# adaliaramon/LambdaGap

Hardware: AMD Instinct MI355X
Metric: boosting iters/sec + AUC, synthetic Higgs-shape 10M×28, 255 bins, 63 leaves (higher is better)
Workload: dtype fp32; 1 GPU; model=gbdt binary, 63 leaves, 255 bins, lr 0.1, global_batch=10000000, seq_len=28, parallelism=dp1, device=AMD GPU (gfx950:sramecc+:xnack-) [frontier engine]

## Files before the change

### src/device/device_learner.hip

```cpp
#include <hip/hip_runtime.h>

#include <algorithm>
#include <chrono>
#include <cmath>
#include <cstdio>
#include <cstdlib>
#include <cstring>
#include <fstream>
#include <map>
#include <memory>
#include <string>
#include <vector>

#include "device/grad_kernels.h"
#include "device/hip_common.h"
#include "device/leaf_kernels.h"
#include "device/metric_eval.h"
#include "device/linear_kernels.h"
#include "device/runtime_internal.h"
#include "device/frontier.h"
#include "device/policy_scan.h"
#include "device/traverse_kernels.h"
#include "device/sample_kernels.h"
#include "device/engine_plan.h"
#include "device/seq_kernels.h"
#include "device/split_scan.h"
#include "device/tree_kernels.h"
#include "learner/forced_splits.h"
#include "learner/linear_solve.h"
#include "learner/parallel_tree_learner.h"
#include "learner/serial_tree_learner.h"
#include "lgap/common.h"
#include "lgap/device_api.h"
#include "lgap/network.h"
#include "lgap/objective.h"
#include "lgap/rank_math.h"
#include "lgap/metric.h"
#include "lgap/split_math.h"

namespace lgap {
namespace device {
namespace {

const char* KernelOverride(const char* key) {
  static const char* const kKeys[] = {"fhist_threads", "hist_lds_kb", "quant_lds32", "part_iters",
                                      "hist_il",       "nibble",      "quant_hist",  "scan_global",
                                      "scan_wave",     "oob_rows",    "select_merge", "part_grid"};
  constexpr int kNumKeys = static_cast<int>(sizeof(kKeys) / sizeof(kKeys[0]));
  thread_local std::string vals[kNumKeys];
  const char* e = std::getenv("LGAP_KERNEL");
  if (e == nullptr) return nullptr;
  const std::string s(e);
  const char* found = nullptr;
  for (size_t p = 0; p < s.size();) {
    size_t q = s.find(',', p);
    if (q == std::string::npos) q = s.size();
    const std::string item = s.substr(p, q - p);
    p = q + 1;
    if (item.empty()) continue;
    const size_t eq = item.find('=');
    const std::string k = item.substr(0, eq);
    int idx = -1;
    for (int i = 0; i < kNumKeys; ++i) idx = k == kKeys[i] ? i : idx;
    if (idx < 0) Log::Fatal("LGAP_KERNEL: unknown key '%s'", k.c_str());
    if (k == key) {
      vals[idx] = eq == std::string::npos ? "1" : item.substr(eq + 1);
      found = vals[idx].c_str();
    }
  }
  return found;
}


using namespace seq;

class DeviceTreeLearner : public TreeLearner {
 public:
  DeviceTreeLearner(const Config* config, const std::string& learner_type, bool routed = false)
      : config_(config), learner_type_(learner_type), routed_(routed) {}

  ~DeviceTreeLearner() override {
    if (fres_host_) (void)hipHostFree(fres_host_);
    if (graph_exec_) (void)hipGraphExecDestroy(graph_exec_);
    for (auto& kv : fgraphs_) (void)hipGraphExecDestroy(kv.second);
    if (fcont_) (void)hipGraphExecDestroy(fcont_);
    if (!fx_peers_.empty()) XgmiClose(fx_local_, &fx_peers_);
    if (fx_local_) (void)hipFree(fx_local_);
    for (auto& ev : pipe_ev_) {
      if (ev) (void)hipEventDestroy(ev);
    }
    if (comm_stream_) (void)hipStreamDestroy(comm_stream_);
    if (stream_) (void)hipStreamDestroy(stream_);
  }

  void Init(const Dataset* train, bool is_constant_hessian) override {
    is_const_hess_ = is_constant_hessian;
    data_ = train;
    N_ = train->num_data();
    F_ = train->num_features();
    G_ = train->num_groups();
    TB_ = train->num_total_bin();
    width_ = train->bin_width();
    stride_dw_ = train->row_stride() / 4;
    tstride_dw_ = stride_dw_;
    if (learner_type_ != "serial" && !CommActive() && !HostStagedDP() && Network::num_machines() > 1) {
      Log::Fatal("Parallel HIP training needs an RCCL communicator (LGBM_DeviceCommInit)");
    }
    plan_in_ = PlanInputs();
    Replan();
    device_id_ = CommExists() ? CommDevice() : std::max(0, config_->gpu_device_id);
    HIP_CHECK(hipSetDevice(device_id_));
    hipDeviceProp_t prop;
    HIP_CHECK(hipGetDeviceProperties(&prop, device_id_));
    device_name_ = std::string(prop.name[0] ? prop.name : "AMD GPU") + " (" + prop.gcnArchName + ")";
    num_cu_ = prop.multiProcessorCount;
    if (!stream_) HIP_CHECK(hipStreamCreateWithFlags(&stream_, hipStreamNonBlocking));

    use_dp_ = config_->gpu_use_dp;
    UploadData();
    linear_ = config_->linear_tree;
    if (linear_) {
      if (!train->has_raw() && F_ > 0) {
        Log::Fatal("linear_tree requires the Dataset to keep raw feature values (construct it with linear_tree=true)");
      }
      const auto& raw = train->raw_values();
      lin_has_nan_ = false;
      for (float v : raw) {
        if (std::isnan(v)) {
          lin_has_nan_ = true;
          break;
// ... 1357 lines not shown
    a.L = L_;
    a.C = fC_;
    a.kmax = fkmax_;
    a.gstart = gstart_.get();
    a.feat = feat_.get();
    a.tiles = tiles_.get();
    a.num_tiles = num_tiles_;
    a.used_bytree = used_bytree_.get();
    a.tp = tparams_.get();
    a.st = fst_;
    a.nodes = fnodes_;
    a.exps = fexps_;
    a.exp_bits = fbits_;
    a.lsum = flsum_;
    a.lout = flout_;
    a.bounds = fbounds_;
    a.key = fkey_;
    a.best = fbest_;
    a.spl = fspl_;
    a.ic = use_ic_ ? fic_ : nullptr;
    a.ic_feat = use_ic_ ? fic_feat_.get() : nullptr;
    a.ic_words = ic_words_;
    a.nstate = fnst_;
    a.leaf_cid = flcid_;
    a.rec = rec_.get();
    a.range_out = range_.get();
    a.slots = fslots_.get();
    a.acc = reinterpret_cast<unsigned long long*>(facc_.get());
    a.hslab = fhslab_.get();
    a.hslab_stride = fhslab_stride_;
    a.hmeta = fhmeta_.get();
    a.red_grid = (num_tiles_ > 1 ? 4 : 2) * num_cu_;
    a.ghmax = ghmax_.get();
    a.sum_mult = plan_.distributed && !ffeature_ ? std::max(1, P_) : 1;
    {
      const char* e = std::getenv("LGAP_FIXED_SUMBOUND");
      a.sum_bound = e == nullptr || std::atoi(e) != 0;
    }
    a.forced = fnum_forced_ > 0 ? fforced_.get() : nullptr;
    a.num_forced = fnum_forced_;
    a.fbest = ffbest_;
    a.fkey = ffkey_;
    a.ckey = fckey_;
    a.cinfo = fcinfo_;
    a.tile_pub = ftile_pub_.get();
    a.bar = bar_.get();
    a.hist_min_rows = HistMinRows();
    a.hist_grid = FrontierHistBlocks();
    a.hist_threads = fhist_threads_;
    if (nib_) {
      a.rowbins = rowbins4_.get();
      a.stride_dw = stride4_dw_;
      a.tiles = ntile_.get();
      a.hist_nib = 1;
    }
    a.part_tile = fpart_tile_;
    a.max_depth = config_->max_depth;
    a.use_monotone = config_->monotone_constraints.empty() ? 0 : 1;
    a.mono_inter = fcbnd_ != nullptr ? 1 : 0;
    a.cbnd = fcbnd_;
    const char* sm = KernelOverride("select_merge");
    a.salive = sm != nullptr && sm[0] == '0' ? nullptr : fsal_;
    a.monotone_penalty = config_->monotone_penalty;
    a.cegb_split = CegbPenalty::Enabled(config_) ? config_->cegb_tradeoff * config_->cegb_penalty_split : 0.0;
    a.max_bin = max_bin_;
    a.cat_p2 = cat_p2_;
    a.use_dp = use_dp_ ? 1 : 0;
    a.ghq = ghq_.get();
    a.qmax = qmax_.get();
    a.quant = QuantHist() && ghq_.size() >= static_cast<size_t>(K_) * N_ ? 1 : 0;
    a.qbins = std::max(2, config_->num_grad_quant_bins);
    a.qconst = is_const_hess_ ? 1 : 0;
    {
      const double rows = static_cast<double>(N_);
      const double gl = a.qbins / 2, hl = a.qconst ? 1 : a.qbins;
      a.qpack = rows * gl < 2147483647.0 && rows * hl < 4294967295.0 ? 1 : 0;
      const int sub = static_cast<int>(std::min(32767.0 / gl, 65535.0 / hl));
      const char* e = KernelOverride("quant_lds32");
      const bool want = e != nullptr ? e[0] != '0' : num_tiles_ == 1;
      a.qsub = a.quant && !use_dp_ && sub >= 2048 && want ? sub : 0;
    }
    a.hist_il = !use_dp_ && a.qsub == 0 ? HistInterleave() : 0;
    {
      const bool fits = kFScanWaves * FrontierScanWaveBytes(max_bin_, cat_p2_) <= 150 * 1024;
      const char* sw = KernelOverride("scan_wave");
      a.scan_wave = fits && !has_cat_ && !a.mono_inter && (F_ >= 64 || (sw != nullptr && sw[0] == '1')) ? 1 : 0;
      a.scan_grid = 512;
    }
    a.e_lo = 0;
    a.e_hi = kFrontierKmax;
    if (plan_.raw_cands && fnuep_.size() > 0) {
      a.cegb_raw = 1;
      a.cegb_tradeoff = config_->cegb_tradeoff;
      a.nkey = fnkey_.get();
      a.ninfo = fninfo_.get();
      a.nuep = fnuep_.get();
      if (plan_.cegb_coupled) {
        a.cegb_coupled = cegb_coupled_.get();
        a.cegb_used = cegb_used_.get();
        a.cegb_epoch = cegb_epoch_.get();
      }
      if (plan_.cegb_lazy) {
        a.cegb_lazy = cegb_lazy_.get();
        a.lazy_bits = lazy_bits_.get();
        a.lazy_words = lazy_words_;
        a.lazy_acc = lazy_acc_.get();
        a.nlazy = fnlazy_.get();
        a.npath = fnpath_.get();
      }
    }
    a.spec_cap = fspec_cap_;
    a.policy = fpolicy_;
    a.stamps = fstamps_.size() ? fstamps_.get() : nullptr;
    a.distributed = plan_.distributed ? 1 : 0;
    a.kcap = fcaps_on_ ? fkcap_.get() : nullptr;
    a.kused = plan_.distributed ? fkused_.get() : nullptr;
    if (plan_.distributed) {
      const double gl = a.qbins / 2, hl = a.qconst ? 1 : a.qbins;
      a.qpack = fglobal_rows_ * gl < 2147483647.0 && fglobal_rows_ * hl < 4294967295.0 ? 1 : 0;
    }
    a.sp = MakeArgs().sp;
    a.bynode = use_bynode_ ? bynode_.get() : nullptr;
    a.byn_draw = frontier_ && plan_.bynode_on_device ? bynode_.get() : nullptr;
    a.byn_mode = fbyn_mode_.size() ? fbyn_mode_.get() : nullptr;
    a.byn_cnt = fbyn_cnt_;
    a.byn_reset = fbyn_reset_;
    a.xrng = config_->extra_trees ? rng_.get() : nullptr;
    if (ffeature_ || fowner_) {
      a.fowned = ffowned_.get();
      a.fpb = ffpb_.get();
      a.vote_P = P_;
      a.vote_rank = rank_;
      a.fown_list = fown_list_.get();
      a.fown_n = fown_n_;
    }
    a.xkb = fkmax_;
    if (fowner_) {
      a.own = 1;
      a.own_P = P_;
      a.own_rank = rank_;
      a.own_w = bbin_;
      a.own_b0 = fown_b0_.get();
      a.acc_recv = facc_recv_.get();
    }
    if (FrontierXg()) {
      a.xg = 1;
      a.xsession = 1;
      a.xc = fxconf_.get();
      if (fowner_ || ffeature_) a.fpb = reinterpret_cast<FPairBest*>(fx_local_ + fxo_fpb_);
      if (fowner_) a.acc_recv = reinterpret_cast<unsigned long long*>(fx_local_ + fxo_recv_);
    }
    if (fvoting_) {
      a.voting = 1;
      a.vote_k = topk_;
      a.vote_P = P_;
      a.vote_rank = rank_;
      a.sp_local = fsp_local_.get();
      a.lsum_loc = flsum_loc_.get();
      a.ltot = fltot_.get();
      a.vrec = fvrec_.get();
      a.velect = fvelect_.get();
      a.vrows = reinterpret_cast<unsigned long long*>(fvrows_.get());
      if (FrontierXg()) {
        a.vrec = reinterpret_cast<VoteRec*>(fx_local_ + fxo_vrec_);
        a.vrows = reinterpret_cast<unsigned long long*>(fx_local_ + fxo_vrows_);
      }
// ... 597 lines not shown
    for (int f = 0; f < F_; ++f) put(out + 8 * static_cast<size_t>(f), dev[f]);
    std::vector<float2> ghd(N_);
    HIP_CHECK(hipMemcpy(ghd.data(), gh_.get(), sizeof(float2) * N_, hipMemcpyDeviceToHost));
    std::vector<double> hg(N_), hh(N_);
    for (int i = 0; i < N_; ++i) {
      hg[i] = ghd[i].x;
      hh[i] = ghd[i].y;
    }
    double sg = 0.0, sh = 0.0;
    for (int i = 0; i < N_; ++i) {
      sg += hg[i];
      sh += hh[i];
    }
    const SplitParams sp = fa.sp;
    SplitParams p0 = sp;
    p0.path_smooth = 0.0;
    const double po = LeafOutputRaw(root_sum.x, root_sum.y, p0, N_, 0.0);
    for (int f = 0; f < F_; ++f) {
      const FeatureInfo& fi = data_->feature(f);
      std::vector<double> full(2 * static_cast<size_t>(fi.num_bin), 0.0);
      for (int i = 0; i < N_; ++i) {
        const uint32_t b = data_->FeatureBin(i, f);
        full[2 * b] += hg[i];
        full[2 * b + 1] += hh[i];
      }
      FeatureScanMeta m;
      m.num_bin = fi.num_bin;
      m.default_bin = fi.default_bin;
      m.missing_type = static_cast<int8_t>(fi.missing);
      m.bin_type = static_cast<int8_t>(fi.bin_type);
      m.monotone = fi.monotone;
      m.penalty = fi.penalty;
      SplitInfo r;
      r.Reset();
      bool ok;
      if (fi.bin_type == BinType::Numerical) {
        ok = FindBestNumerical(full.data(), m, sp, sg, sh, N_, po, LeafBounds(), &r);
      } else {
        std::vector<int> order(fi.num_bin);
        ok = FindBestCategorical(full.data(), m, sp, sg, sh, N_, po, LeafBounds(), order.data(), &r);
      }
      r.feature = ok ? f : -1;
      if (!ok) r.gain = kMinScore;
      put(ref + 8 * static_cast<size_t>(f), r);
    }
  }

  void TestFrontierHist(const float* g, const float* h, const int* rows, const int* offsets, int k, double* out,
                        uint16_t* levels) {
    if (!frontier_) Log::Fatal("TestFrontierHist: the frontier engine is not enabled for this configuration");
    if (k < 1 || k > fkmax_) Log::Fatal("TestFrontierHist: %d subsets (1..%d)", k, fkmax_);
    const int total = offsets[k];
    if (idx_[3].size() < static_cast<size_t>(total)) idx_[3].Resize(total);
    K_ = 1;
    DeviceSetGradients(g, h, 1);
    TreeParams* tp = pin_tp_.Get(1);
    std::memset(tp, 0, sizeof(TreeParams));
    tp->root_buf = -1;
    tp->root_count = tp->root_gcount = N_;
    tp->spec_alpha = 1.f;
    HIP_CHECK(hipMemcpyAsync(tparams_.get(), tp, sizeof(TreeParams), hipMemcpyHostToDevice, stream_));
    float bnd[4] = {0.f, 0.f, 0.f, 0.f};
    double sg = 0.0, sh = 0.0;
    for (int i = 0; i < N_; ++i) {
      bnd[0] = std::max(bnd[0], std::fabs(g[i]));
      bnd[1] = std::max(bnd[1], std::fabs(h[i]));
      sg += std::fabs(static_cast<double>(g[i]));
      sh += std::fabs(static_cast<double>(h[i]));
    }
    bnd[2] = std::nextafter(static_cast<float>(sg * (1.0 + 0x1p-20)), INFINITY);
    bnd[3] = std::nextafter(static_cast<float>(sh * (1.0 + 0x1p-20)), INFINITY);
    unsigned* hm = pin_max_.Get(4);
    std::memcpy(hm, bnd, 16);
    HIP_CHECK(hipMemcpyAsync(ghmax_.get(), hm, 16, hipMemcpyHostToDevice, stream_));
    if (config_->use_quantized_grad) QuantizeGradients(0);
    idx_[3].Upload(rows, total, stream_);
    FState st;
    std::memset(&st, 0, sizeof(st));
    st.round = 1;
    st.k = k;
    st.kx = k;
    st.num_leaves = 1;
    std::vector<FExp> ex(k);
    for (int e = 0; e < k; ++e) {
      std::memset(&ex[e], 0, sizeof(FExp));
      ex[e].h_buf = 3;
      ex[e].h_start = offsets[e];
      ex[e].h_count = offsets[e + 1] - offsets[e];
      ex[e].forced = -1;
    }
    HIP_CHECK(hipMemcpyAsync(fst_, &st, sizeof(FState), hipMemcpyHostToDevice, stream_));
    HIP_CHECK(hipMemcpyAsync(fexps_, ex.data(), sizeof(FExp) * k, hipMemcpyHostToDevice, stream_));
    facc_.Zero(stream_);
    FArgs fa = MakeFArgs();
    LaunchFrontierHist(fa, FrontierHistLds(), stream_);
    const int pw = fa.quant && fa.qpack ? 1 : 2;
    std::vector<unsigned long long> acc(static_cast<size_t>(k) * pw * TB_);
    HIP_CHECK(hipMemcpyAsync(acc.data(), facc_.get(), acc.size() * 8, hipMemcpyDeviceToHost, stream_));
    if (fa.quant && levels != nullptr) HIP_CHECK(hipMemcpyAsync(levels, ghq_.get(), sizeof(uint16_t) * N_, hipMemcpyDeviceToHost, stream_));
    HIP_CHECK(hipStreamSynchronize(stream_));
    facc_.Zero(stream_);
    HIP_CHECK(hipStreamSynchronize(stream_));
    constexpr double k62 = 4611686018427387904.0;
    const float sb2 = fa.sum_bound ? bnd[2] : INFINITY, sb3 = fa.sum_bound ? bnd[3] : INFINITY;
    const double ig = fa.quant ? 1.0 : std::ldexp(1.0, -FixedPointExp(k62, N_, bnd[0], sb2));
    const double ih = fa.quant ? 1.0 : std::ldexp(1.0, -FixedPointExp(k62, N_, bnd[1], sb3));
    for (int e = 0; e < k; ++e) {
      for (int b = 0; b < TB_; ++b) {
        const size_t o = (static_cast<size_t>(e) * TB_ + b) * pw;
        long long qg, qh;
        if (pw == 1) {
          const unsigned long long hs = acc[o] & 0xFFFFFFFFull;
          qg = static_cast<long long>(acc[o] - hs) >> 32;
          qh = static_cast<long long>(hs);
        } else {
          qg = static_cast<long long>(acc[o]);
          qh = static_cast<long long>(acc[o + 1]);
        }
        out[(static_cast<size_t>(e) * TB_ + b) * 2] = static_cast<double>(qg) * ig;
        out[(static_cast<size_t>(e) * TB_ + b) * 2 + 1] = static_cast<double>(qh) * ih;
      }
    }
  }

  bool TestQuantize(const float* g, const float* h, int num_class, int rounds, float* out_gh, uint16_t* out_levels,
                    uint32_t* out_qmax, float* out_true) {
    if (!config_->use_quantized_grad) Log::Fatal("TestQuantize: use_quantized_grad is not set");
    if (num_class < 1 || rounds < 1) Log::Fatal("TestQuantize: %d classes, %d rounds", num_class, rounds);
    K_ = num_class;
    const size_t n = static_cast<size_t>(N_);
    for (int r = 0; r < rounds; ++r) {
      DeviceSetGradients(g, h, num_class);
      for (int c = 0; c < num_class; ++c) {
        QuantizeGradients(c);
        const size_t o = (static_cast<size_t>(r) * num_class + c) * n;
        HIP_CHECK(hipMemcpyAsync(out_gh + 2 * o, gh_.get() + static_cast<size_t>(c) * n, sizeof(float2) * n,
                                 hipMemcpyDeviceToHost, stream_));
        if (QuantHist()) {
          HIP_CHECK(hipMemcpyAsync(out_levels + o, ghq_.get() + static_cast<size_t>(c) * n, sizeof(uint16_t) * n,
                                   hipMemcpyDeviceToHost, stream_));
        }
        HIP_CHECK(hipMemcpyAsync(out_qmax + 2 * (static_cast<size_t>(r) * num_class + c), qmax_.get(), 8,
                                 hipMemcpyDeviceToHost, stream_));
        if (config_->quant_train_renew_leaf) {
          HIP_CHECK(hipMemcpyAsync(out_true + 2 * o, gh_true_.get(), sizeof(float2) * n, hipMemcpyDeviceToHost, stream_));
        }
        HIP_CHECK(hipStreamSynchronize(stream_));
      }
    }
    return QuantHist();
  }

  void TestFrontierPartition(const int* rows, const int* offsets, int k, const int* feats, const int* thr,
                             const int* dleft, const uint32_t* catbits, int* out_rows, int* out_left, int* exp_rows,
                             int* exp_left) {
    if (!frontier_) Log::Fatal("TestFrontierPartition: the frontier engine is not enabled for this configuration");
    if (k < 1 || k > fkmax_ || 3 * k > fC_) Log::Fatal("TestFrontierPartition: %d parents (1..%d)", k, fkmax_);
    const int total = offsets[k];
    if (total > N_) Log::Fatal("TestFrontierPartition: %d rows over the subsets (at most %d)", total, N_);
    FState st;
    HIP_CHECK(hipMemcpyAsync(&st, fst_, sizeof(FState), hipMemcpyDeviceToHost, stream_));
    HIP_CHECK(hipStreamSynchronize(stream_));
    idx_[0].Upload(rows, total, stream_);
    std::vector<FExp> ex(k);
    std::vector<uint32_t> bits(static_cast<size_t>(fkmax_) * kMaxCatWords, 0u);
    int tiles = 0;
    for (int e = 0; e < k; ++e) {
      const int f = feats[e];
      if (f < 0 || f >= F_) Log::Fatal("TestFrontierPartition: feature %d", f);
      const FeatureInfo& fi = data_->feature(f);
      FExp& x = ex[e];
// ... 1421 lines not shown
```

### src/device/frontier.h

```cpp
#pragma once

#include <hip/hip_runtime.h>

#include <cstdint>

#include "device/frontier_shape.h"
#include "device/tree_kernels.h"
#include "lgap/split_math.h"

namespace lgap {
namespace device {

#ifndef LGAP_FRONTIER_BUFS
#define LGAP_FRONTIER_BUFS 4
#endif
constexpr int kFrontierBufs = LGAP_FRONTIER_BUFS;
constexpr int kFrontierIdx = kFrontierBufs + 1;
constexpr int kFrontierRoundCap = 64;

__host__ __device__ inline int FixedPointExp(double limit, double rows, float vmax, float vsum) {
  double b = rows * static_cast<double>(vmax);
  if (static_cast<double>(vsum) < b) b = static_cast<double>(vsum);
  if (!(b > 0.0)) return 0;
  int e;
// ... 44 lines not shown
  int rescan;
};

struct FState {
  int round;
  int k;
  int kx;
  int total_tiles;
  int done;
  unsigned epoch;
  int num_leaves, num_splits;
  int cid_next;
  int blocked;
  int spec;
  long long used_rows, waste_rows;
  int forced_next;
  int byn;
  unsigned byn_rng;
  int nsal;
};

struct FArgs {
  const uint32_t* rowbins;
  const uint8_t* colbins;
  const float2* gh;
  int* idx[kFrontierIdx];
  int N, stride_dw, width, num_groups, TB, F, L, C, kmax;
  const int* gstart;
  const DevFeature* feat;
  const HistTile* tiles;
  int num_tiles;
  const uint8_t* used_bytree;
  const TreeParams* tp;
  FState* st;
  FNode* nodes;
  FExp* exps;
  uint32_t* exp_bits;
  double2* lsum;
  double* lout;
  LeafBounds* bounds;
  SplitKey* key;
  SplitInfo* best;
  uint8_t* spl;
  unsigned long long* ic;
  const unsigned long long* ic_feat;
  int ic_words;
  uint8_t* nstate;
  int* leaf_cid;
  SplitRec* rec;
  LeafRange* range_out;
  double* slots;
  unsigned long long* acc;
  unsigned long long* hslab;
  size_t hslab_stride;
  long long* hmeta;
  int red_grid;
  int own, own_P, own_rank, own_w;
  const int* own_b0;
  unsigned long long* acc_recv;
  int xkb;
  const int* fown_list;
  int fown_n;
  const unsigned* ghmax;
  int sum_mult;
  int sum_bound;
  const FForced* forced;
  int num_forced;
  SplitInfo* fbest;
  SplitKey* fkey;
  const uint16_t* ghq;
  const unsigned* qmax;
  int quant;
  int qpack;
  int qbins, qconst;
  int qsub;
  SplitKey* ckey;
  SplitInfo* cinfo;
  unsigned long long* tile_pub;
  unsigned* bar;
  int part_selfcount;
  int hist_min_rows, hist_grid;
  int hist_threads;
  int hist_il;
  int scan_wave;
  int scan_grid;
  int hist_nib;
  int part_tile;
  int max_depth, use_monotone;
  int mono_inter;
  LeafBounds* cbnd;
  int* salive;
  double monotone_penalty;
  double cegb_split;
  const double* cegb_coupled;
  double cegb_tradeoff;
  uint8_t* cegb_used;
  unsigned* cegb_epoch;
  SplitKey* nkey;
  SplitInfo* ninfo;
  int* nuep;
  int cegb_raw;
  const double* cegb_lazy;
  uint32_t* lazy_bits;
  int lazy_words;
  int* lazy_acc;
  int* nlazy;
  uint32_t* npath;
  int max_bin, cat_p2;
  int use_dp;
  int spec_cap;
  int policy;
  int distributed;
  const int* kcap;
  int* kused;
  unsigned long long* stamps;
  int e_lo, e_hi;
  int voting;
  int vote_k, vote_P, vote_rank;
  const SplitParams* sp_local;
  double2* lsum_loc;
  unsigned long long* ltot;
  VoteRec* vrec;
  int* velect;
  unsigned long long* vrows;
  const uint8_t* fowned;
  const uint8_t* bynode;
  uint8_t* byn_draw;
  const uint8_t* byn_mode;
  int byn_cnt;
  int byn_reset;
  unsigned* xrng;
  struct FPairBest* fpb;
  SplitParams sp;
  int xg;
  unsigned xsession;
  const struct FXConf* xc;
};

struct FXConf {
  char* peer[kMaxXRanks];
  size_t o_recv, o_fpb, o_root, o_flag;
  size_t o_vrec, o_vrows;
  unsigned* ep;
  unsigned* cnt;
  unsigned long long timeout;
  int P, rank;
  int fault;
  int pad;
};

constexpr int kFXHist = 0, kFXCand = 1, kFXRoot = 2, kFXVote = 3, kFXVRows = 4, kFXTest = 5, kFXKinds = 6;
struct FXRoot {
  double g, h;
  unsigned m[4];
};

struct FResultHdr {
  FState st;
  unsigned bar[4];
  double lout0;
  int kused[kFrontierRoundCap];
};
__host__ __device__ inline size_t FrontierResultRecOffset() { return (sizeof(FResultHdr) + 15) & ~size_t(15); }
__host__ __device__ inline size_t FrontierResultRangeOffset(int L) {
  return FrontierResultRecOffset() + ((sizeof(SplitRec) * static_cast<size_t>(L > 1 ? L - 1 : 1) + 15) & ~size_t(15));
}
// ... 31 lines not shown
```

### src/device/frontier_kernels.hip

```cpp
#include <hip/hip_runtime.h>

#include <algorithm>
#include <cstdint>

#include "device/frontier.h"
#include "device/hip_common.h"
#include "device/split_scan.h"
#include "lgap/split_math.h"

namespace lgap {
namespace device {
namespace {

constexpr int kFPartThreads = 256;
constexpr int kFScanThreads = 256;
constexpr int kFSelThreads = 1024;
#ifndef LGAP_FHIST_R
#define LGAP_FHIST_R 16
#endif

__device__ __forceinline__ int FRowAt(const FArgs& a, int buf, int pos) { return buf < 0 ? pos : a.idx[buf][pos]; }

__device__ __forceinline__ uint32_t FColBin(const FArgs& a, int g, int row) {
  const size_t o = static_cast<size_t>(g) * a.N + row;
// ... 170 lines not shown
    r.start = 0;
    r.count = tp.root_count;
    r.gcount = tp.root_gcount;
    r.depth = 0;
    r.parent = -1;
    r.left = -1;
    r.fidx = a.num_forced > 0 ? 0 : -1;
    a.nodes[0] = r;
    FExp x;
    x.parent = -1;
    x.left = -1;
    x.depth = -1;
    x.tile0 = x.ntiles = 0;
    x.src_buf = tp.root_buf;
    x.start = 0;
    x.count = tp.root_count;
    x.dst_buf = 0;
    x.group = x.offset = x.num_bin = x.mfb = x.default_bin = x.missing = x.thr = x.default_left = x.is_cat = 0;
    x.skip = 0;
    x.smaller = 0;
    x.larger = -1;
    x.h_buf = tp.root_buf;
    x.h_start = 0;
    x.h_count = tp.root_count;
    x.forced = -1;
    x.feature = -1;
    x.last = 0;
    x.rescan = 0;
    a.exps[0] = x;
    a.bounds[0] = LeafBounds();
    if (a.cbnd) a.cbnd[0] = LeafBounds();
    if (a.ic) {
      for (int w = 0; w < a.ic_words; ++w) a.ic[w] = ~0ull;
    }
    a.leaf_cid[0] = 0;
    a.lout[0] = 0.0;
  }
  for (int i = t; i < a.C; i += blockDim.x) a.nstate[i] = 0;
  for (int f = t; f < a.F; f += blockDim.x) a.spl[f] = 1;
}

__global__ __launch_bounds__(256) void k_f_init(FArgs a) { FInitTree(a); }

constexpr int kRootStatsF = 6;
__device__ __forceinline__ double FRootFold(int i, double x, double y) { return i == 2 || i == 3 ? fmax(x, y) : x + y; }
__global__ __launch_bounds__(256) void k_f_init_root(FArgs a, const double* __restrict__ root_part, int nblocks,
                                                     unsigned* __restrict__ ghmax) {
  __shared__ double sh[kRootStatsF][256 / 64];
  double v[kRootStatsF] = {0.0, 0.0, 0.0, 0.0, 0.0, 0.0};
  for (int b = threadIdx.x; b < nblocks; b += blockDim.x) {
#pragma unroll
    for (int j = 0; j < kRootStatsF; ++j) v[j] = FRootFold(j, v[j], root_part[kRootStatsF * b + j]);
  }
  FInitTree(a);
#pragma unroll
  for (int j = 0; j < kRootStatsF; ++j) {
    if (j == 2 || j == 3) {
#pragma unroll
      for (int o = 32; o > 0; o >>= 1) v[j] = fmax(v[j], __shfl_xor(v[j], o, kWave));
    } else {
      v[j] = WaveSum(v[j]);
    }
  }
  const int w = threadIdx.x >> 6;
  if ((threadIdx.x & 63) == 0) {
#pragma unroll
    for (int j = 0; j < kRootStatsF; ++j) sh[j][w] = v[j];
  }
  __syncthreads();
  if (threadIdx.x == 0) {
    for (int i = 1; i < static_cast<int>(blockDim.x / 64); ++i) {
#pragma unroll
      for (int j = 0; j < kRootStatsF; ++j) v[j] = FRootFold(j, v[j], sh[j][i]);
    }
    a.lsum[0] = make_double2(v[0], v[1]);
    ghmax[0] = __float_as_uint(static_cast<float>(v[2]));
    ghmax[1] = __float_as_uint(static_cast<float>(v[3]));
    ghmax[2] = __float_as_uint(__double2float_ru(v[4] * (1.0 + 0x1p-20)));
    ghmax[3] = __float_as_uint(__double2float_ru(v[5] * (1.0 + 0x1p-20)));
  }
}

constexpr int kFHistR2 = LGAP_FHIST_R / 2;
__device__ __forceinline__ void FHistFirstRows(const FArgs& a, const HistTile& tile, int buf, int start, int rb, int re,
                                               int* rn) {
  const int tpr = tile.d1 - tile.d0;
  const int rpi = blockDim.x / tpr;
  const int myr = threadIdx.x / tpr;
  const int* idx = buf < 0 ? nullptr : a.idx[buf] + start;
  const int base = buf < 0 ? start : 0;
#pragma unroll
  for (int j = 0; j < kFHistR2; ++j) {
    const int p = rb + myr + j * rpi;
    rn[j] = myr < rpi && p < re ? (idx ? idx[p] : base + p) : -1;
  }
}

template <int W, int MODE>
__device__ __forceinline__ void FHistRows(const FArgs& a, const HistTile& tile, int buf, int start, int rb, int re,
                                          const int* gst, unsigned long long* hist, float sg, float sh, double dsg,
                                          double dsh, uint32_t* hist32 = nullptr, int il_gp = 0,
                                          const int* first_rows = nullptr) {
  const int tpr = tile.d1 - tile.d0;
  const int rpi = blockDim.x / tpr;
  const int myr = threadIdx.x / tpr;
  const int myd = threadIdx.x - myr * tpr;
  if (myr >= rpi) return;
  constexpr int per = W == 0 ? 8 : 4 / W;
  constexpr int R = LGAP_FHIST_R;
  const int dw = tile.d0 + myd;
  const int gfirst = dw * per;
  int go[per], gsh[per];
  const int rot = (MODE == 0 || MODE == 2) && il_gp > 0 ? (myr & (per - 1)) : 0;
#pragma unroll
  for (int kk = 0; kk < per; ++kk) {
    int gv = -1, sv = 0;
#pragma unroll
    for (int k = 0; k < per; ++k) {
      if (k == ((kk + rot) & (per - 1))) {
        const int gl = gfirst + k - tile.g0;
        gv = gfirst + k < tile.g1 ? (il_gp > 0 ? gl : gst[gl]) : -1;
        sv = (W == 0 ? 4 : W == 1 ? 8 : 16) * k;
      }
    }
    go[kk] = gv;
    gsh[kk] = sv;
  }
  const float2* gh = a.gh + static_cast<size_t>(a.tp->cls) * a.N;
  const uint16_t* ghq = MODE >= 2 ? a.ghq + static_cast<size_t>(a.tp->cls) * a.N : nullptr;
  const int* idx = buf < 0 ? nullptr : a.idx[buf] + start;
  const int base = buf < 0 ? start : 0;
  constexpr int R2 = R / 2;
  static_assert(R2 == kFHistR2, "first-chunk prefetch width");
  const int step = rpi * R2;
  auto load_rows = [&](int p0, int* rows) {
#pragma unroll
    for (int j = 0; j < R2; ++j) {
      const int p = p0 + j * rpi;
      rows[j] = p < re ? (idx ? idx[p] : base + p) : -1;
    }
  };
  auto load_data = [&](const int* rows, uint32_t* word, float2* v, uint32_t* q) {
#pragma unroll
    for (int j = 0; j < R2; ++j) {
      word[j] = rows[j] >= 0 ? a.rowbins[static_cast<size_t>(rows[j]) * a.stride_dw + dw] : 0u;
      if (MODE >= 2) q[j] = rows[j] >= 0 ? ghq[rows[j]] : 0u;
      else v[j] = rows[j] >= 0 ? gh[rows[j]] : make_float2(0.f, 0.f);
    }
  };
  int rn[R2];
  uint32_t word[R2], q[R2];
  float2 v[R2];
  if (first_rows != nullptr) {
#pragma unroll
    for (int j = 0; j < R2; ++j) rn[j] = first_rows[j];
  } else {
    load_rows(rb + myr, rn);
  }
  load_data(rn, word, v, q);
  load_rows(rb + myr + step, rn);
  for (int p0 = rb + myr; p0 < re; p0 += step) {
    uint32_t wn[R2], qn[R2];
    float2 vn[R2];
    load_data(rn, wn, vn, qn);
    load_rows(p0 + 2 * step, rn);
#pragma unroll
    for (int j = 0; j < R2; ++j) {
      unsigned long long pg = 0ull, ph = 0ull;
      uint32_t p32 = 0u;
      if (MODE == 3) {
        p32 = (static_cast<uint32_t>(static_cast<int32_t>(static_cast<int8_t>(q[j] >> 8))) << 16) + (q[j] & 0xFFu);
      } else if (MODE == 2) {
        const long long ig = static_cast<int8_t>(q[j] >> 8);
        pg = (static_cast<unsigned long long>(ig) << 32) + (q[j] & 0xFFu);
      } else if (MODE == 0) {
        const long long ig = __float2int_rn(v[j].x * sg);
        const long long ih = __float2int_rn(v[j].y * sh);
        pg = (static_cast<unsigned long long>(ig) << 32) + static_cast<unsigned long long>(ih);
      } else {
        pg = static_cast<unsigned long long>(__double2ll_rn(static_cast<double>(v[j].x) * dsg));
        ph = static_cast<unsigned long long>(__double2ll_rn(static_cast<double>(v[j].y) * dsh));
      }
#pragma unroll
      for (int k = 0; k < per; ++k) {
        const uint32_t b = (word[j] >> gsh[k]) & (W == 0 ? 0xFu : W == 1 ? 0xFFu : 0xFFFFu);
        if (b != 0u && go[k] >= 0) {
          const int o = il_gp > 0 ? static_cast<int>(b) * il_gp + go[k] : go[k] + static_cast<int>(b);
          if (MODE == 3) {
            atomicAdd(&hist32[o], p32);
          } else if (MODE != 1) {
            atomicAdd(&hist[o], pg);
          } else {
            atomicAdd(&hist[2 * o], pg);
            atomicAdd(&hist[2 * o + 1], ph);
          }
        }
      }
    }
#pragma unroll
    for (int j = 0; j < R2; ++j) {
      word[j] = wn[j];
      q[j] = qn[j];
      v[j] = vn[j];
    }
  }
}

struct FChunkSrc {
  int cnt, buf, start;
};
__device__ __forceinline__ FChunkSrc FHistChunkLoad(const FArgs& a) {
  FChunkSrc c{0, -1, 0};
  const int t = threadIdx.x;
  if (t < kFrontierKmax) {
    const FExp& x = a.exps[t];
    c.cnt = x.skip ? 0 : x.h_count;
    c.buf = x.h_buf;
    c.start = x.h_start;
  }
  return c;
}
__device__ __forceinline__ void FHistChunks(const FArgs& a, int k, const FChunkSrc& src, int* cnt, int* nb, int* inc) {
  const int t = threadIdx.x;
  *cnt = t < k && t >= a.e_lo && t < a.e_hi ? src.cnt : 0;
  const int total = WaveSum(*cnt);
  const int ke = WaveSum(*cnt > 0 ? 1 : 0);
  const int slots = max(max(1, a.hist_grid / 2), a.hist_grid - ke);
  const int c = max(a.hist_min_rows, (total + slots - 1) / slots);
  *nb = (*cnt + c - 1) / c;
  *inc = WaveInclusiveScan(*nb);
}

template <int W, int MODE, int THREADS>
__global__ __launch_bounds__(THREADS) void k_f_hist(FArgs a) {
  extern __shared__ __align__(8) unsigned char lds_raw[];
  __shared__ int s_e, s_rb, s_re, s_buf, s_start;
  const FState* sp = a.st;
  const int t = threadIdx.x;
  const FChunkSrc csrc = FHistChunkLoad(a);
  const HistTile tile = a.tiles[blockIdx.y];
  const int ng0 = tile.g1 - tile.g0;
  const int gst0 = t < ng0 ? a.gstart[tile.g0 + t] : 0;
  int EG, EH;
  GlobalScaleExp(a, &EG, &EH);
  if (sp->done) return;
  const int k = sp->k;
  const int rnd = sp->round;
  FStamp(a, rnd, kFStampHist, 0);
  if (t < 64) {
    int cnt, nb, inc;
    FHistChunks(a, k, csrc, &cnt, &nb, &inc);
    const int bx = static_cast<int>(blockIdx.x);
    const bool mine = nb > 0 && bx >= inc - nb && bx < inc;
    const unsigned long long m = __ballot(mine);
    if (mine) {
      const int j = bx - (inc - nb);
      const int chunk = (cnt + nb - 1) / nb;
      s_e = t;
      s_rb = j * chunk;
      s_re = min(cnt, (j + 1) * chunk);
      s_buf = csrc.buf;
      s_start = csrc.start;
    }
    if (t == 0 && m == 0ull) s_e = -1;
  }
  __syncthreads();
  const int e = s_e;
  if (e < 0) return;
  FStampMax(a, rnd, kFStampHist, 4);
  const int rb = s_rb, re = s_re, buf = s_buf, start = s_start;
  const int pw = a.quant && a.qpack ? 1 : 2;
  const double dsg = ldexp(1.0, EG), dsh = ldexp(1.0, EH);
  if (a.ltot != nullptr && blockIdx.y == 0) {
    __shared__ unsigned long long s_tot[2];
    if (t < 2) s_tot[t] = 0ull;
    __syncthreads();
    long long sg = 0, sh = 0;
    for (int p = rb + t; p < re; p += blockDim.x) {
      const int row = FRowAt(a, buf, start + p);
      if (a.quant) {
        const uint32_t qv = a.ghq[static_cast<size_t>(a.tp->cls) * a.N + row];
        sg += static_cast<int8_t>(qv >> 8);
        sh += static_cast<long long>(qv & 0xFFu);
      } else {
        const float2 v = a.gh[static_cast<size_t>(a.tp->cls) * a.N + row];
        sg += __double2ll_rn(static_cast<double>(v.x) * dsg);
        sh += __double2ll_rn(static_cast<double>(v.y) * dsh);
      }
    }
    if (sg) atomicAdd(&s_tot[0], static_cast<unsigned long long>(sg));
    if (sh) atomicAdd(&s_tot[1], static_cast<unsigned long long>(sh));
    __syncthreads();
    if (t < 2 && s_tot[t]) atomicAdd(&a.ltot[2 * e + t], s_tot[t]);
  }
  if (tile.direct) {
    if (a.own && e >= a.xkb) return;
    int* gst = reinterpret_cast<int*>(lds_raw);
    for (int g = t; g < ng0; g += blockDim.x) gst[g] = g == t ? gst0 : a.gstart[tile.g0 + g];
    __syncthreads();
    const int tpr = tile.d1 - tile.d0;
    const int rpi = blockDim.x / tpr;
    const int myr = t / tpr, myd = t - myr * tpr;
    if (myr >= rpi) return;
    constexpr int per = W == 0 ? 8 : 4 / W;
    const int dw = tile.d0 + myd;
    const float2* gh = a.gh + static_cast<size_t>(a.tp->cls) * a.N;
    for (int p = rb + myr; p < re; p += rpi) {
      const int row = FRowAt(a, buf, start + p);
      const uint32_t word = a.rowbins[static_cast<size_t>(row) * a.stride_dw + dw];
      unsigned long long qg, qh;
      if (MODE >= 2) {
        const uint32_t qv = a.ghq[static_cast<size_t>(a.tp->cls) * a.N + row];
        qg = static_cast<unsigned long long>(static_cast<long long>(static_cast<int8_t>(qv >> 8)));
        qh = qv & 0xFFu;
        if (a.qpack) qg = (qg << 32) + qh, qh = 0ull;
      } else {
        const float2 v = gh[row];
        qg = static_cast<unsigned long long>(__double2ll_rn(static_cast<double>(v.x) * dsg));
        qh = static_cast<unsigned long long>(__double2ll_rn(static_cast<double>(v.y) * dsh));
      }
#pragma unroll
      for (int kk = 0; kk < per; ++kk) {
        const uint32_t b = W == 0   ? ((word >> (4 * kk)) & 0xFu)
                           : W == 1 ? ((word >> (8 * kk)) & 0xFFu)
                                    : ((word >> (16 * kk)) & 0xFFFFu);
        const int g = dw * per + kk;
        if (b != 0u && g < tile.g1) {
          unsigned long long* o = FAccPtr(a, e, gst[g - tile.g0] + static_cast<int>(b), pw);
          if (a.xg && a.own) {
            if (qg) FXAdd(o, qg);
            if (qh) FXAdd(o + 1, qh);
          } else {
            if (qg) atomicAdd(o, qg);
            if (qh) atomicAdd(o + 1, qh);
          }
        }
      }
    }
    if (a.xg && a.own) __builtin_amdgcn_s_waitcnt(0);
    return;
  }
  const double rows_in_block = static_cast<double>(re - rb > 0 ? re - rb : 1);
  constexpr double k30 = 1073741824.0;
  const float sbg = a.sum_bound ? __uint_as_float(a.ghmax[2]) : INFINITY;
  const float sbh = a.sum_bound ? __uint_as_float(a.ghmax[3]) : INFINITY;
  const int bg = FixedPointExp(k30, rows_in_block, __uint_as_float(a.ghmax[0]), sbg);
  const int bh = FixedPointExp(k30, rows_in_block, __uint_as_float(a.ghmax[1]), sbh);
  const float sg = ldexpf(1.f, bg), sh = ldexpf(1.f, bh);
  const int ng = tile.g1 - tile.g0;
  const int il_gp = (MODE == 0 || MODE == 2) && a.hist_il && tile.pad > 0 && (buf < 0 || a.hist_il > 1) ? ((ng + 15) & ~15) : 0;
  const int words = il_gp > 0 ? tile.pad * il_gp : (MODE != 1 ? tile.nbins : 2 * tile.nbins);
  unsigned long long* hist = reinterpret_cast<unsigned long long*>(lds_raw);
  uint32_t* hist32 = reinterpret_cast<uint32_t*>(hist + words);
  int* gst = reinterpret_cast<int*>(MODE == 3 ? reinterpret_cast<unsigned long long*>(hist32 + ((tile.nbins + 1) & ~1))
                                              : hist + words);
  unsigned long long* packed = il_gp > 0 ? reinterpret_cast<unsigned long long*>(gst + ((ng + 1) & ~1)) : nullptr;
  int first_rows[kFHistR2];
  if (MODE != 3) FHistFirstRows(a, tile, buf, start, rb, re, first_rows);
  for (int i = t; i < words; i += blockDim.x) hist[i] = 0ull;
  if (MODE == 3) {
    for (int i = t; i < tile.nbins; i += blockDim.x) hist32[i] = 0u;
  }
  for (int g = t; g < ng0; g += blockDim.x) gst[g] = (g == t ? gst0 : a.gstart[tile.g0 + g]) - tile.bin0;
  __syncthreads();
  FStamp(a, rnd, kFStampHist, 1);
  if (MODE == 3) {
    for (int sb = rb; sb < re; sb += a.qsub) {
      const int se = min(re, sb + a.qsub);
      FHistRows<W, MODE>(a, tile, buf, start, sb, se, gst, hist, sg, sh, dsg, dsh, hist32);
      __syncthreads();
      for (int i = t; i < tile.nbins; i += blockDim.x) {
        const uint32_t x = hist32[i];
        if (x == 0u) continue;
        hist32[i] = 0u;
        const uint32_t hs = x & 0xFFFFu;
        const long long gs = static_cast<int32_t>(x - hs) >> 16;
        hist[i] += (static_cast<unsigned long long>(gs) << 32) + hs;
      }
      __syncthreads();
    }
  } else {
    FHistRows<W, MODE>(a, tile, buf, start, rb, re, gst, hist, sg, sh, dsg, dsh, nullptr, il_gp, first_rows);
    __syncthreads();
  }
  if (il_gp > 0) {
    for (int sl = t; sl < words; sl += blockDim.x) {
      const int b = sl / il_gp, gl = sl - b * il_gp;
      if (gl >= ng) continue;
      const int nb = (gl + 1 < ng ? gst[gl + 1] : tile.nbins) - gst[gl];
      if (b < nb) packed[gst[gl] + b] = hist[sl];
    }
    __syncthreads();
  }
  FStamp(a, rnd, kFStampHist, 2);
  FStampMax(a, rnd, kFStampHist, 5);
  const int sw = MODE == 1 ? 2 : 1;
  unsigned long long* prow = a.hslab + static_cast<size_t>(blockIdx.x) * a.hslab_stride + static_cast<size_t>(sw) * tile.bin0;
  const unsigned long long* src = il_gp > 0 ? packed : hist;
  for (int j = t; j < sw * tile.nbins; j += blockDim.x) prow[j] = src[j];
  if (MODE == 0 && t == 0) {
    a.hmeta[blockIdx.x] = static_cast<long long>((static_cast<unsigned long long>(static_cast<unsigned>(bh)) << 32) |
                                                 static_cast<unsigned>(bg));
  }
  FStamp(a, rnd, kFStampHist, 3);
  FStampMax(a, rnd, kFStampHist, 6);
  FStampEnd(a, rnd, kFStampHist);
}

constexpr int kRedThreads = 256;
constexpr int kRedRows = 16;
constexpr int kRedMaxTiles = 256;

template <int MODE, bool XG>
__global__ __launch_bounds__(kRedThreads) void k_f_reduce(FArgs a) {
  __shared__ int s_nb[kFrontierKmax], s_b0[kFrontierKmax], s_w0[kFrontierKmax + 1];
  __shared__ int s_tc[kRedMaxTiles + 1];
  __shared__ int s_wc[kRedThreads / 64];
  __shared__ int s_tb0[kRedMaxTiles], s_tnb[kRedMaxTiles];
  const FState* sp = a.st;
  const int t = threadIdx.x, lane = t & 63, wv = t >> 6;
  const FChunkSrc csrc = FHistChunkLoad(a);
  int tch = 0;
  if (t < a.num_tiles) {
    const HistTile ty = a.tiles[t];
    tch = ty.direct ? 0 : (ty.nbins + kRedThreads - 1) / kRedThreads;
    s_tb0[t] = ty.bin0;
    s_tnb[t] = ty.nbins;
  }
  int EG, EH;
  GlobalScaleExp(a, &EG, &EH);
  const bool xhist = XG && a.xg && a.own;
  const unsigned xep = xhist ? *a.xc->ep : 0u;
  if (sp->done) return;
  const int k = sp->k;
  const int tinc = WaveInclusiveScan(tch);
  if (lane == 63) s_wc[wv] = tinc;
  __syncthreads();
  int woff = 0;
  for (int q = 0; q < wv; ++q) woff += s_wc[q];
  if (t < a.num_tiles) s_tc[t] = woff + tinc - tch;
  if (t == 0) {
    int tot = 0;
    for (int q = 0; q < kRedThreads / 64; ++q) tot += s_wc[q];
    s_tc[a.num_tiles] = tot;
  }
  if (t < 64) {
    int cnt, nb, inc;
    FHistChunks(a, k, csrc, &cnt, &nb, &inc);
    if (t < kFrontierKmax) {
      s_nb[t] = nb;
      s_b0[t] = inc - nb;
    }
// ... 3192 lines not shown
```

Before: 421.0 iters/s.

## Specialize frontier histogram row loop by address width, index mode and interleave

```diff
diff --git a/src/device/device_learner.hip b/src/device/device_learner.hip
--- a/src/device/device_learner.hip
+++ b/src/device/device_learner.hip
@@ -45,7 +45,8 @@
 const char* KernelOverride(const char* key) {
   static const char* const kKeys[] = {"fhist_threads", "hist_lds_kb", "quant_lds32", "part_iters",
                                       "hist_il",       "nibble",      "quant_hist",  "scan_global",
-                                      "scan_wave",     "oob_rows",    "select_merge", "part_grid"};
+                                      "scan_wave",     "oob_rows",    "select_merge", "part_grid",
+                                      "fhist_addr",    "fhist_contig"};
   constexpr int kNumKeys = static_cast<int>(sizeof(kKeys) / sizeof(kKeys[0]));
   thread_local std::string vals[kNumKeys];
   const char* e = std::getenv("LGAP_KERNEL");
@@ -1569,6 +1570,16 @@
     }
     a.hist_il = !use_dp_ && a.qsub == 0 ? HistInterleave() : 0;
     {
+      const double rows = static_cast<double>(N_), stride_b = 4.0 * a.stride_dw;
+      const bool fits32 = rows * std::max(stride_b, 8.0) < 4294967296.0;
+      const bool fits24 = fits32 && N_ <= (1 << 24) && stride_b < 16777216.0;
+      a.hist_addr = fits24 ? 24 : fits32 ? 32 : 64;
+      if (const char* e = KernelOverride("fhist_addr")) {
+        const int want = std::atoi(e);
+        if (want == 64 || (want == 32 && fits32)) a.hist_addr = want;
+      }
+    }
+    {
       const bool fits = kFScanWaves * FrontierScanWaveBytes(max_bin_, cat_p2_) <= 150 * 1024;
       const char* sw = KernelOverride("scan_wave");
       a.scan_wave = fits && !has_cat_ && !a.mono_inter && (F_ >= 64 || (sw != nullptr && sw[0] == '1')) ? 1 : 0;
@@ -2332,11 +2343,22 @@
     st.kx = k;
     st.num_leaves = 1;
     std::vector<FExp> ex(k);
+    const char* ck = KernelOverride("fhist_contig");
+    const bool contig = ck != nullptr && ck[0] == '1';
     for (int e = 0; e < k; ++e) {
       std::memset(&ex[e], 0, sizeof(FExp));
       ex[e].h_buf = 3;
       ex[e].h_start = offsets[e];
       ex[e].h_count = offsets[e + 1] - offsets[e];
+      if (contig && ex[e].h_count > 0) {
+        const int* r = rows + offsets[e];
+        bool asc = true;
+        for (int i = 1; i < ex[e].h_count && asc; ++i) asc = r[i] == r[0] + i;
+        if (asc) {
+          ex[e].h_buf = -1;
+          ex[e].h_start = r[0];
+        }
+      }
       ex[e].forced = -1;
     }
     HIP_CHECK(hipMemcpyAsync(fst_, &st, sizeof(FState), hipMemcpyHostToDevice, stream_));
diff --git a/src/device/frontier.h b/src/device/frontier.h
--- a/src/device/frontier.h
+++ b/src/device/frontier.h
@@ -150,6 +150,7 @@
   int hist_min_rows, hist_grid;
   int hist_threads;
   int hist_il;
+  int hist_addr;
   int scan_wave;
   int scan_grid;
   int hist_nib;
diff --git a/src/device/frontier_kernels.hip b/src/device/frontier_kernels.hip
--- a/src/device/frontier_kernels.hip
+++ b/src/device/frontier_kernels.hip
@@ -276,110 +276,153 @@
 }
 
 constexpr int kFHistR2 = LGAP_FHIST_R / 2;
-__device__ __forceinline__ void FHistFirstRows(const FArgs& a, const HistTile& tile, int buf, int start, int rb, int re,
-                                               int* rn) {
+struct FHistRowIds {
+  int r[kFHistR2];
+};
+__device__ __forceinline__ FHistRowIds FHistFirstRows(const FArgs& a, const HistTile& tile, int buf, int start, int rb,
+                                                      int re) {
   const int tpr = tile.d1 - tile.d0;
   const int rpi = blockDim.x / tpr;
   const int myr = threadIdx.x / tpr;
-  const int* idx = buf < 0 ? nullptr : a.idx[buf] + start;
-  const int base = buf < 0 ? start : 0;
-#pragma unroll
-  for (int j = 0; j < kFHistR2; ++j) {
-    const int p = rb + myr + j * rpi;
-    rn[j] = myr < rpi && p < re ? (idx ? idx[p] : base + p) : -1;
-  }
-}
-
-template <int W, int MODE>
-__device__ __forceinline__ void FHistRows(const FArgs& a, const HistTile& tile, int buf, int start, int rb, int re,
-                                          const int* gst, unsigned long long* hist, float sg, float sh, double dsg,
-                                          double dsh, uint32_t* hist32 = nullptr, int il_gp = 0,
-                                          const int* first_rows = nullptr) {
+  FHistRowIds rn;
+#pragma unroll
+  for (int j = 0; j < kFHistR2; ++j) rn.r[j] = 0;
+  if (buf >= 0 && re > rb) {
+    const int* idx = a.idx[buf] + start;
+#pragma unroll
+    for (int j = 0; j < kFHistR2; ++j) rn.r[j] = idx[min(rb + myr + j * rpi, re - 1)];
+  }
+  return rn;
+}
+
+struct FHistSet {
+  uint32_t word[kFHistR2], q[kFHistR2];
+  float2 v[kFHistR2];
+};
+template <bool B>
+struct FHistFlag {
+  static constexpr bool value = B;
+};
+template <int V>
+struct FHistInt {
+  static constexpr int value = V;
+};
+
+template <int W, int MODE, bool IL, bool IDX, int AB>
+__device__ __forceinline__ void FHistRowsT(const FArgs& a, const HistTile& tile, const int* idx, int base, int rb,
+                                           int re, const int* gst, unsigned long long* hist, float sg, float sh,
+                                           double dsg, double dsh, uint32_t* hist32, int il_gp,
+                                           const FHistRowIds& first_rows) {
   const int tpr = tile.d1 - tile.d0;
   const int rpi = blockDim.x / tpr;
   const int myr = threadIdx.x / tpr;
   const int myd = threadIdx.x - myr * tpr;
-  if (myr >= rpi) return;
+  if (myr >= rpi || re <= rb) return;
   constexpr int per = W == 0 ? 8 : 4 / W;
-  constexpr int R = LGAP_FHIST_R;
+  constexpr int bits = W == 0 ? 4 : W == 1 ? 8 : 16;
+  constexpr int R2 = kFHistR2;
   const int dw = tile.d0 + myd;
   const int gfirst = dw * per;
-  int go[per], gsh[per];
-  const int rot = (MODE == 0 || MODE == 2) && il_gp > 0 ? (myr & (per - 1)) : 0;
+  int go[per];
+  uint32_t gsh[per], gwd[per];
+  const int rot = IL ? (myr & (per - 1)) : 0;
 #pragma unroll
   for (int kk = 0; kk < per; ++kk) {
-    int gv = -1, sv = 0;
+    int gv = 0;
+    uint32_t sv = 0, wv = 0;
 #pragma unroll
     for (int k = 0; k < per; ++k) {
       if (k == ((kk + rot) & (per - 1))) {
         const int gl = gfirst + k - tile.g0;
-        gv = gfirst + k < tile.g1 ? (il_gp > 0 ? gl : gst[gl]) : -1;
-        sv = (W == 0 ? 4 : W == 1 ? 8 : 16) * k;
+        const bool in = gfirst + k < tile.g1;
+        gv = in ? (IL ? gl : gst[gl]) : 0;
+        wv = in ? bits : 0;
+        sv = bits * k;
       }
     }
     go[kk] = gv;
     gsh[kk] = sv;
-  }
-  const float2* gh = a.gh + static_cast<size_t>(a.tp->cls) * a.N;
-  const uint16_t* ghq = MODE >= 2 ? a.ghq + static_cast<size_t>(a.tp->cls) * a.N : nullptr;
-  const int* idx = buf < 0 ? nullptr : a.idx[buf] + start;
-  const int base = buf < 0 ? start : 0;
-  constexpr int R2 = R / 2;
-  static_assert(R2 == kFHistR2, "first-chunk prefetch width");
+    gwd[kk] = wv;
+  }
+  const char* rbp = reinterpret_cast<const char*>(a.rowbins);
+  const char* ghp = reinterpret_cast<const char*>(a.gh + static_cast<size_t>(a.tp->cls) * a.N);
+  const char* gqp = MODE >= 2 ? reinterpret_cast<const char*>(a.ghq + static_cast<size_t>(a.tp->cls) * a.N) : nullptr;
+  const uint32_t stride_b = 4u * a.stride_dw, dwb = 4u * dw;
+  const uint32_t lane_w = myr * stride_b + dwb, lane_g = 8u * myr, lane_q = 2u * myr, lane_i = 4u * myr;
   const int step = rpi * R2;
-  auto load_rows = [&](int p0, int* rows) {
+  auto load_row = [&](int row, uint32_t* word, float2* v, uint32_t* q) {
+    if constexpr (AB == 64) {
+      *word = a.rowbins[static_cast<size_t>(row) * a.stride_dw + dw];
+      if constexpr (MODE >= 2) *q = reinterpret_cast<const uint16_t*>(gqp)[row];
+      else *v = reinterpret_cast<const float2*>(ghp)[row];
+    } else {
+      const uint32_t r = static_cast<uint32_t>(row);
+      const uint32_t o = (AB == 24 ? __umul24(r, stride_b) : r * stride_b) + dwb;
+      *word = *reinterpret_cast<const uint32_t*>(rbp + o);
+      if constexpr (MODE >= 2) *q = *reinterpret_cast<const uint16_t*>(gqp + (r << 1));
+      else *v = *reinterpret_cast<const float2*>(ghp + (r << 3));
+    }
+  };
+  auto load_rows = [&](auto full, int P, int* rows) {
+    if constexpr (IDX) {
+#pragma unroll
+      for (int j = 0; j < R2; ++j) {
+        if constexpr (decltype(full)::value && AB != 64) {
+          const uint32_t vo = 4u * static_cast<uint32_t>(P) + lane_i;
+          rows[j] = *reinterpret_cast<const int*>(reinterpret_cast<const char*>(idx + j * rpi) + vo);
+        } else if constexpr (decltype(full)::value) {
+          rows[j] = *reinterpret_cast<const int*>(reinterpret_cast<const char*>(idx + P + j * rpi) + lane_i);
+        } else {
+          rows[j] = idx[min(P + myr + j * rpi, re - 1)];
+        }
+      }
+    }
+  };
+  auto load_data = [&](auto full, int P, const int* rows, FHistSet& s) {
 #pragma unroll
     for (int j = 0; j < R2; ++j) {
-      const int p = p0 + j * rpi;
-      rows[j] = p < re ? (idx ? idx[p] : base + p) : -1;
+      if constexpr (!IDX && decltype(full)::value && AB != 64) {
+        const uint32_t r0 = static_cast<uint32_t>(base + P);
+        const size_t rj = static_cast<size_t>(j * rpi);
+        s.word[j] = *reinterpret_cast<const uint32_t*>(rbp + rj * stride_b + (r0 * stride_b + lane_w));
+        if constexpr (MODE >= 2) s.q[j] = *reinterpret_cast<const uint16_t*>(gqp + rj * 2 + (r0 * 2u + lane_q));
+        else s.v[j] = *reinterpret_cast<const float2*>(ghp + rj * 8 + (r0 * 8u + lane_g));
+      } else if constexpr (!IDX && decltype(full)::value) {
+        const size_t r0 = static_cast<size_t>(base + P + j * rpi);
+        s.word[j] = *reinterpret_cast<const uint32_t*>(rbp + r0 * stride_b + lane_w);
+        if constexpr (MODE >= 2) s.q[j] = *reinterpret_cast<const uint16_t*>(gqp + r0 * 2 + lane_q);
+        else s.v[j] = *reinterpret_cast<const float2*>(ghp + r0 * 8 + lane_g);
+      } else {
+        const int p = P + myr + j * rpi;
+        const int row = IDX ? rows[j] : base + min(p, re - 1);
+        load_row(row, &s.word[j], &s.v[j], &s.q[j]);
+        if constexpr (!decltype(full)::value) s.word[j] = p < re ? s.word[j] : 0u;
+      }
     }
   };
-  auto load_data = [&](const int* rows, uint32_t* word, float2* v, uint32_t* q) {
-#pragma unroll
-    for (int j = 0; j < R2; ++j) {
-      word[j] = rows[j] >= 0 ? a.rowbins[static_cast<size_t>(rows[j]) * a.stride_dw + dw] : 0u;
-      if (MODE >= 2) q[j] = rows[j] >= 0 ? ghq[rows[j]] : 0u;
-      else v[j] = rows[j] >= 0 ? gh[rows[j]] : make_float2(0.f, 0.f);
-    }
-  };
-  int rn[R2];
-  uint32_t word[R2], q[R2];
-  float2 v[R2];
-  if (first_rows != nullptr) {
-#pragma unroll
-    for (int j = 0; j < R2; ++j) rn[j] = first_rows[j];
-  } else {
-    load_rows(rb + myr, rn);
-  }
-  load_data(rn, word, v, q);
-  load_rows(rb + myr + step, rn);
-  for (int p0 = rb + myr; p0 < re; p0 += step) {
-    uint32_t wn[R2], qn[R2];
-    float2 vn[R2];
-    load_data(rn, wn, vn, qn);
-    load_rows(p0 + 2 * step, rn);
+  auto add_rows = [&](const FHistSet& s) {
 #pragma unroll
     for (int j = 0; j < R2; ++j) {
       unsigned long long pg = 0ull, ph = 0ull;
       uint32_t p32 = 0u;
       if (MODE == 3) {
-        p32 = (static_cast<uint32_t>(static_cast<int32_t>(static_cast<int8_t>(q[j] >> 8))) << 16) + (q[j] & 0xFFu);
+        p32 = (static_cast<uint32_t>(static_cast<int32_t>(static_cast<int8_t>(s.q[j] >> 8))) << 16) + (s.q[j] & 0xFFu);
       } else if (MODE == 2) {
-        const long long ig = static_cast<int8_t>(q[j] >> 8);
-        pg = (static_cast<unsigned long long>(ig) << 32) + (q[j] & 0xFFu);
+        const long long ig = static_cast<int8_t>(s.q[j] >> 8);
+        pg = (static_cast<unsigned long long>(ig) << 32) + (s.q[j] & 0xFFu);
       } else if (MODE == 0) {
-        const long long ig = __float2int_rn(v[j].x * sg);
-        const long long ih = __float2int_rn(v[j].y * sh);
+        const long long ig = __float2int_rn(s.v[j].x * sg);
+        const long long ih = __float2int_rn(s.v[j].y * sh);
         pg = (static_cast<unsigned long long>(ig) << 32) + static_cast<unsigned long long>(ih);
       } else {
-        pg = static_cast<unsigned long long>(__double2ll_rn(static_cast<double>(v[j].x) * dsg));
-        ph = static_cast<unsigned long long>(__double2ll_rn(static_cast<double>(v[j].y) * dsh));
+        pg = static_cast<unsigned long long>(__double2ll_rn(static_cast<double>(s.v[j].x) * dsg));
+        ph = static_cast<unsigned long long>(__double2ll_rn(static_cast<double>(s.v[j].y) * dsh));
       }
 #pragma unroll
       for (int k = 0; k < per; ++k) {
-        const uint32_t b = (word[j] >> gsh[k]) & (W == 0 ? 0xFu : W == 1 ? 0xFFu : 0xFFFFu);
-        if (b != 0u && go[k] >= 0) {
-          const int o = il_gp > 0 ? static_cast<int>(b) * il_gp + go[k] : go[k] + static_cast<int>(b);
+        const uint32_t b = __builtin_amdgcn_ubfe(s.word[j], gsh[k], gwd[k]);
+        if (b != 0u) {
+          const int o = IL ? static_cast<int>(__umul24(b, static_cast<uint32_t>(il_gp))) + go[k] : go[k] + static_cast<int>(b);
           if (MODE == 3) {
             atomicAdd(&hist32[o], p32);
           } else if (MODE != 1) {
@@ -391,13 +434,75 @@
         }
       }
     }
-#pragma unroll
-    for (int j = 0; j < R2; ++j) {
-      word[j] = wn[j];
-      q[j] = qn[j];
-      v[j] = vn[j];
-    }
-  }
+  };
+  constexpr FHistFlag<true> kFull;
+  constexpr FHistFlag<false> kChecked;
+  FHistSet s0, s1;
+  int rn[R2];
+  if constexpr (MODE != 3) {
+#pragma unroll
+    for (int j = 0; j < R2; ++j) rn[j] = first_rows.r[j];
+  } else {
+    load_rows(kChecked, rb, rn);
+  }
+  load_data(kChecked, rb, rn, s0);
+  load_rows(kChecked, rb + step, rn);
+  int P = rb;
+  auto iter = [&](auto full, const FHistSet& cur, FHistSet& nxt) {
+    load_data(full, P + step, rn, nxt);
+    load_rows(full, P + 2 * step, rn);
+    add_rows(cur);
+    P += step;
+  };
+  const int len = re - rb;
+  const int niter = (len + step - 1) / step;
+  const int nfull = max(0, len / step - 2);
+  int i = 0;
+  if (nfull > 0) {
+    for (;;) {
+      iter(kFull, s0, s1);
+      if (++i == nfull) {
+        s0 = s1;
+        break;
+      }
+      iter(kFull, s1, s0);
+      if (++i == nfull) break;
+    }
+  }
+  for (; i < niter; ++i) {
+    iter(kChecked, s0, s1);
+    s0 = s1;
+  }
+}
+
+template <int W, int MODE>
+__device__ __forceinline__ void FHistRows(const FArgs& a, const HistTile& tile, int buf, int start, int rb, int re,
+                                          const int* gst, unsigned long long* hist, float sg, float sh, double dsg,
+                                          double dsh, uint32_t* hist32, int il_gp, const FHistRowIds& first_rows) {
+  const int* idx = buf < 0 ? nullptr : a.idx[buf] + start;
+  const int base = buf < 0 ? start : 0;
+  auto run = [&](auto il, auto ix, auto ab) {
+    FHistRowsT<W, MODE, decltype(il)::value, decltype(ix)::value, decltype(ab)::value>(
+        a, tile, idx, base, rb, re, gst, hist, sg, sh, dsg, dsh, hist32, il_gp, first_rows);
+  };
+  constexpr FHistFlag<true> yes;
+  constexpr FHistFlag<false> no;
+  using A24 = FHistInt<24>;
+  using A32 = FHistInt<32>;
+  using A64 = FHistInt<64>;
+  if constexpr (MODE == 0 || MODE == 2) {
+    if (il_gp > 0) {
+      if (idx == nullptr && a.hist_addr == 64) run(yes, no, A64());
+      else if (idx == nullptr) run(yes, no, A32());
+      else run(yes, yes, A64());
+      return;
+    }
+  }
+  if (idx == nullptr && a.hist_addr == 64) run(no, no, A64());
+  else if (idx == nullptr) run(no, no, A32());
+  else if (a.hist_addr == 24) run(no, yes, A24());
+  else if (a.hist_addr == 32) run(no, yes, A32());
+  else run(no, yes, A64());
 }
 
 struct FChunkSrc {
@@ -462,7 +567,8 @@
   const int e = s_e;
   if (e < 0) return;
   FStampMax(a, rnd, kFStampHist, 4);
-  const int rb = s_rb, re = s_re, buf = s_buf, start = s_start;
+  const int rb = __builtin_amdgcn_readfirstlane(s_rb), re = __builtin_amdgcn_readfirstlane(s_re);
+  const int buf = __builtin_amdgcn_readfirstlane(s_buf), start = __builtin_amdgcn_readfirstlane(s_start);
   const int pw = a.quant && a.qpack ? 1 : 2;
   const double dsg = ldexp(1.0, EG), dsh = ldexp(1.0, EH);
   if (a.ltot != nullptr && blockIdx.y == 0) {
@@ -549,8 +655,8 @@
   int* gst = reinterpret_cast<int*>(MODE == 3 ? reinterpret_cast<unsigned long long*>(hist32 + ((tile.nbins + 1) & ~1))
                                               : hist + words);
   unsigned long long* packed = il_gp > 0 ? reinterpret_cast<unsigned long long*>(gst + ((ng + 1) & ~1)) : nullptr;
-  int first_rows[kFHistR2];
-  if (MODE != 3) FHistFirstRows(a, tile, buf, start, rb, re, first_rows);
+  FHistRowIds first_rows{};
+  if (MODE != 3) first_rows = FHistFirstRows(a, tile, buf, start, rb, re);
   for (int i = t; i < words; i += blockDim.x) hist[i] = 0ull;
   if (MODE == 3) {
     for (int i = t; i < tile.nbins; i += blockDim.x) hist32[i] = 0u;
@@ -561,7 +667,7 @@
   if (MODE == 3) {
     for (int sb = rb; sb < re; sb += a.qsub) {
       const int se = min(re, sb + a.qsub);
-      FHistRows<W, MODE>(a, tile, buf, start, sb, se, gst, hist, sg, sh, dsg, dsh, hist32);
+      FHistRows<W, MODE>(a, tile, buf, start, sb, se, gst, hist, sg, sh, dsg, dsh, hist32, 0, first_rows);
       __syncthreads();
       for (int i = t; i < tile.nbins; i += blockDim.x) {
         const uint32_t x = hist32[i];
```

Result: no change. 419.7 iters/s (-0.3%).
